# secastel/phaser

Measured on AMD Instinct MI355X. Metric: het-SNP allele calls/sec + phased variants/sec, whole-genome RNA-seq, 1→8 GPUs, higher is better.
Workload: dtype u8/int32; 1 GPU; configs[2]: whole genome (22 autosomes), one GTEx-shape RNA-seq sample, 79999998 records x 76 bp, 1499988 het SNPs, one shard per chromosome; chromosomes LPT-assigned to GPUs by record count; records=79999998, het_snps=1499988

## Files before the change

phaser_amd/csrc/phz_map.hip:

```cpp
#include "phz_internal.h"
#include "phz_lbound.h"
#include <stdlib.h>
#include <string.h>

namespace {

#ifndef PHZ_MAP_WIN
#define PHZ_MAP_WIN 512
#endif
#ifndef PHZ_CIG_X2
#define PHZ_CIG_X2 5
#endif
#ifndef PHZ_CAND_X4
#define PHZ_CAND_X4 3
#endif
constexpr int MAP_WIN = PHZ_MAP_WIN;

constexpr uint32_t OP_M = 0, OP_I = 1, OP_D = 2, OP_N = 3, OP_S = 4, OP_EQ = 7, OP_X = 8, OP_G = 9;

struct MapArgs {
    const int32_t *pos;
    const uint32_t *cigar_off, *cigar, *seq_off;
    const uint8_t *seq2, *qual;
    const uint8_t *bq;
// ... 441 lines not shown
        const int j = k * MAP_BLOCK + tid;
        const bool ok = j < nr;
        rpos_[k] = ok ? a.pos[r0 + j] : 0;
        soff_[k] = ok ? a.seq_off[r0 + j] : 0;
        coff_[k] = a.cigar_off[r0 + (ok ? j : nr)];
    }
    const uint32_t coff_end = a.cigar_off[r0 + nr];
    int v_first = 0x7fffffff;
    if (tid < vw.wlen) { const int idx = vw.w0 + tid; v_first = idx < a.nv ? a.vpos[idx] : 0x7fffffff; }
    uint32_t cg[3] = {0, 0, 0};
#pragma unroll
    for (int u = 0; u < 3; u++) { const uint32_t j = (uint32_t)tid + (uint32_t)u * MAP_BLOCK; if (j < cnt_w) cg[u] = a.cigar[cw.c_begin + j]; }
#pragma unroll
    for (int k = 0; k < RPT; k++) {
        const int j = k * MAP_BLOCK + tid;
        s_pos[j] = rpos_[k]; s_soff[j] = soff_[k]; s_coff[j] = coff_[k];
    }
    if (tid == 0) { s_coff[TILE] = coff_end; s_ncand = 0; s_ncx = 0; s_nlong = 0; s_nins = 0; }
    if (tid < TILE / 32) s_poison[tid] = 0;
    const int wdepth = window_depth(vw.wlen);
#ifdef PHZ_FILL_ALL
    const int wfill = MAP_WIN;
#else
    const int wfill = (1 << wdepth) > vw.wlen ? (1 << wdepth) : vw.wlen;
#endif
    if (tid < wfill) s_vpos[tid] = v_first;
    for (int j = tid + MAP_BLOCK; j < wfill; j += MAP_BLOCK) {
        const int idx = vw.w0 + j;
        s_vpos[j] = (j < vw.wlen && idx < a.nv) ? a.vpos[idx] : 0x7fffffff;
    }
#pragma unroll
    for (int u = 0; u < 3; u++) { const uint32_t j = (uint32_t)tid + (uint32_t)u * MAP_BLOCK; if (j < cnt_w) s_cig[j] = cg[u]; }
    for (uint32_t j = (uint32_t)tid + 3u * MAP_BLOCK; j < cnt_w; j += MAP_BLOCK) s_cig[j] = a.cigar[cw.c_begin + j];
    __syncthreads();
    PHZ_STAMP(1);
    CandBuf cb;
    cb.key = s_key; cb.var = s_var; cb.x0 = s_x0; cb.ins = s_ins; cb.n = &s_ncand; cb.nins = &s_nins; cb.cap = CAND; cb.w0 = vw.w0;
    const long long cover = (long long)s_pos[nr - 1] + MAP_COVER;

    uint32_t c0_[RPT], c1_[RPT];
    int base_[RPT], n_[RPT];
    uint32_t vmask_[RPT], codes_[RPT];
    bool fast_[RPT];
#pragma unroll
    for (int k = 0; k < RPT; k++) {
        const int j = k * MAP_BLOCK + tid;
        c0_[k] = s_coff[j]; c1_[k] = s_coff[j + 1];
        base_[k] = 0; n_[k] = 0; vmask_[k] = 0; codes_[k] = 0; fast_[k] = false;
    }
    const bool walk_on = !(a.dbg & 8);
    int len_[RPT]; bool one_[RPT];
#pragma unroll
    for (int k = 0; k < RPT; k++) {
        const int j = k * MAP_BLOCK + tid;
        one_[k] = false; len_[k] = 0;
        const uint32_t d = c0_[k] - cw.c_begin;
        if (j < nr && walk_on && complete && c1_[k] - c0_[k] == 1 && d < (uint32_t)CIG) {
            const uint32_t w = s_cig[d];
            const uint32_t op = w & 15;
            len_[k] = (int)(w >> 4);
            one_[k] = (op == OP_M || op == OP_EQ || op == OP_X) && (long long)rpos_[k] + len_[k] <= cover;
        }
    }
    constexpr int GROUP = 64 / (2 * RPT);
    int target = 0x7fffffff;
#pragma unroll
    for (int k = 0; k < RPT; k++) {
        const int e = wave_max(one_[k] ? rpos_[k] + len_[k] : (int)0x80000000);
        const int first = __builtin_amdgcn_readfirstlane(rpos_[k]);
        if ((lane / GROUP) == 2 * k) target = first;
        if ((lane / GROUP) == 2 * k + 1) target = e;
    }
    const int bound = lds_lower_bound(s_vpos, wdepth, target);
#pragma unroll
    for (int k = 0; k < RPT; k++) {
        const int j = k * MAP_BLOCK + tid;
        const int lo = __builtin_amdgcn_readlane(bound, 2 * k * GROUP), hi = __builtin_amdgcn_readlane(bound, (2 * k + 1) * GROUP);
        if (one_[k]) {
            const int pos = rpos_[k], end = pos + len_[k];
            if (hi - lo <= 24) {
                int below = 0, c = 0;
                for (int e = lo; e < hi; e++) {
                    const int vp = s_vpos[e];
                    below += vp < pos ? 1 : 0;
                    c += (vp >= pos && vp < end) ? 1 : 0;
                }
                if (c <= 8) { fast_[k] = true; base_[k] = lo + below; n_[k] = c; }
            } else {
                const int base = lds_lower_bound(s_vpos, wdepth, pos);
                int c = 0;
                while (base + c < vw.wlen && s_vpos[base + c] < end && c <= 8) c++;
                if (c <= 8) { fast_[k] = true; base_[k] = base; n_[k] = c; }
            }
        }
        if (j < nr && walk_on && !fast_[k]) {
            if (s_coff[j + 1] - s_coff[j] > 3u) s_cx[TILE - 1 - atomicAdd(&s_nlong, 1)] = (uint16_t)j;
            else s_cx[atomicAdd(&s_ncx, 1)] = (uint16_t)j;
        }
    }
    uint32_t pre_q[RPT], pre_s[RPT];
#pragma unroll
    for (int k = 0; k < RPT; k++) {
        pre_q[k] = 0; pre_s[k] = 0;
        if (fast_[k] && n_[k] > 0 && !(a.dbg & 1)) {
            const uint32_t soff = s_soff[k * MAP_BLOCK + tid];
            const int x = s_vpos[base_[k]] - rpos_[k];
            if (PHZ_ONEPLANE(a)) pre_q[k] = a.bq[(size_t)soff * 4 + x];
            else { pre_q[k] = a.qual[(size_t)soff * 4 + x]; pre_s[k] = PHZ_SEQ_BYTE(a, soff, x); }
        }
    }
    PHZ_STAMP(2);
    __syncthreads();
    PHZ_STAMP(3);
    const int nshort = walk_on ? s_ncx : 0;
    const int ncx = (walk_on && !(a.dbg & 256)) ? nshort + s_nlong : 0;
    const bool lean_on = complete && !(a.dbg & 32);
    bool redo_any = false;
    for (int t = tid; t < ncx; t += MAP_BLOCK) {
        const int ts = t < nshort ? t : TILE - 1 - (t - nshort);
        const int j = s_cx[ts];
        const bool done = lean_on && walk_lean(s_vpos, vw.wlen, wdepth, vw.w0, s_cig, cw.c_begin, (uint32_t)CIG, cb, s_poison, j, s_pos[j], s_coff[j], s_coff[j + 1], cover, a.dbg);
        if (!done) { s_cx[ts] = (uint16_t)(j | 0x8000); redo_any = true; }
    }
    const bool redo = __syncthreads_or(redo_any ? 1 : 0) != 0;
#pragma unroll
    for (int k = 0; k < RPT; k++) s_mask[k * MAP_BLOCK + tid] = 0;
    if (redo) {
        for (int t = tid; t < ncx; t += MAP_BLOCK) {
            const int jf = s_cx[t < nshort ? t : TILE - 1 - (t - nshort)];
            if (jf & 0x8000) { const int j = jf & 0x7FFF; walk_read<0>(a, vw, cw, cb, j, r0 + j, a.pos[r0 + j], s_coff[j], s_coff[j + 1], 0, 0, 0); }
        }
    }
    __syncthreads();
    PHZ_STAMP(4);
    const int ncand = s_ncand;
    const bool fb = ncand > CAND;
    uint32_t cq = 0, cs = 0; int cx_off = -1;
    if (!fb && tid < ncand && !(a.dbg & 1)) {
        const uint32_t key = s_key[tid];
        if ((key & 0xFF) == 7u) {
            const uint32_t x0 = cand_x0(cb, tid);
            cx_off = x0 != 0xFFFFFFFFu ? (int)x0 : (int)(cand_x1(cb, tid, key) >> 12);
            const uint32_t soff = s_soff[key >> 16];
            if (PHZ_ONEPLANE(a)) cq = a.bq[(size_t)soff * 4 + cx_off];
            else { cq = a.qual[(size_t)soff * 4 + cx_off]; cs = PHZ_SEQ_BYTE(a, soff, cx_off); }
        }
    }
#pragma unroll
    for (int k = 0; k < RPT; k++) {
        if (!fast_[k]) continue;
        const int j = k * MAP_BLOCK + tid;
        const uint32_t soff = s_soff[j];
        for (int o = 0; o < n_[k]; o++) {
            const int x = s_vpos[base_[k] + o] - rpos_[k];
            int sy;
            if (a.dbg & 1) sy = x & 3;
            else if (o == 0) {
                if (PHZ_ONEPLANE(a)) sy = sym_from_bq(a, soff, x, pre_q[k]);
                else {
                    const uint32_t q = pre_q[k], sb = (pre_s[k] >> (2 * (x & 3))) & 3;
                    sy = (int)(q & 0x7f) < a.baseq ? 4 : ((q & 0x80) ? (sb == 0 ? 4 : 5) : (int)sb);
                }
            } else sy = masked_base(a, soff, x);
            if (sy != 4) { vmask_[k] |= 1u << o; codes_[k] |= (uint32_t)(sy < 4 ? sy : 4) << (4 * o); }
        }
    }
    int cnt[RPT], off[RPT];
    if (!fb) {
        for (int e = tid; e < ncand; e += MAP_BLOCK) {
            uint32_t key = s_key[e];
            const int j = (int)(key >> 16);
            int code = (int)(key & 0xFF);
            if ((key & 0x8000u) && ((s_poison[j >> 5] >> (j & 31)) & 1u)) code = -1;
            else if (code == 7) {
                const uint32_t x0 = cand_x0(cb, e);
                const int x = x0 != 0xFFFFFFFFu ? (int)x0 : (int)(cand_x1(cb, e, key) >> 12);
                int sy;
                if (a.dbg & 1) sy = x & 3;
                else if (e == tid && cx_off == x) {
                    if (PHZ_ONEPLANE(a)) sy = sym_from_bq(a, s_soff[j], x, cq);
                    else {
                        const uint32_t sb = (cs >> (2 * (x & 3))) & 3;
                        sy = (int)(cq & 0x7f) < a.baseq ? 4 : ((cq & 0x80) ? (sb == 0 ? 4 : 5) : (int)sb);
                    }
                } else sy = masked_base(a, s_soff[j], x);
                code = sy < 4 ? sy : (sy == 4 ? -1 : 4);
            }
            if (code >= 0) {
                atomicOr(&s_mask[j], 1u << ((key >> 8) & 31));
                s_key[e] = (key & 0xFFFFFF00u) | (uint32_t)code;
            } else {
                s_key[e] = key | 0xFFu;
            }
        }
        __syncthreads();
#pragma unroll
        for (int k = 0; k < RPT; k++) cnt[k] = fast_[k] ? __popc(vmask_[k]) : __popc(s_mask[k * MAP_BLOCK + tid]);
    } else {
#pragma unroll
        for (int k = 0; k < RPT; k++) {
            const int j = k * MAP_BLOCK + tid;
            cnt[k] = fast_[k] ? __popc(vmask_[k])
                              : (j < nr && walk_on ? walk_read<1>(a, vw, cw, cb, j, r0 + j, rpos_[k], c0_[k], c1_[k], s_soff[j], 0, 0) : 0);
        }
    }
    PHZ_STAMP(5);
    const int T = block_scan<MAP_BLOCK, RPT>(cnt, off, s_wsum, lane, wave);
#pragma unroll
    for (int k = 0; k < RPT; k++) s_coff[k * MAP_BLOCK + tid] = (uint32_t)off[k];
    if (tid == 0) {
        a.tile_total[gtile] = T;
        uint32_t first = (uint32_t)(gtile * (int64_t)a.slot_cap);
        int room = a.slot_cap;
        if (T > a.slot_cap) {
            const OvfArea ov = *bt.ovf;
            const unsigned long long at = atomicAdd(ov.cursor, (unsigned long long)T);
            const bool fits = at + (unsigned long long)T <= (unsigned long long)ov.cap;
            if (fits) { first = (uint32_t)(ov.base + (long long)at); room = T; }
            ov.tile_first[gtile] = fits ? first : 0xFFFFFFFFu;
        }
        s_ncx = (int)first; s_nlong = room;
    }
    __syncthreads();
    PHZ_STAMP(6);
    if (a.dbg & 2) return;
    const int64_t slot0 = (int64_t)(uint32_t)s_ncx;
    const int slot_n = s_nlong;
#pragma unroll
    for (int k = 0; k < RPT; k++) {
        const int j = k * MAP_BLOCK + tid;
        if (fast_[k]) {
            int o2 = off[k];
            for (int o = 0; o < n_[k]; o++) {
                if (!((vmask_[k] >> o) & 1)) continue;
                if (o2 < slot_n) {
                    const int64_t g = slot0 + o2;
                    stage_put(a.stage, a.side, a.slots, g, (uint32_t)(vw.w0 + base_[k] + o), (uint32_t)(s_vpos[base_[k] + o] - rpos_[k]), 0u,
                              (uint32_t)j, (codes_[k] >> (4 * o)) & 15u);
                }
                o2++;
            }
        } else if (fb && cnt[k] > 0) {
            walk_read<2>(a, vw, cw, cb, j, r0 + j, rpos_[k], c0_[k], c1_[k], s_soff[j], slot0 + off[k], slot0 + slot_n);
        }
    }
    if (!fb) {
        for (int e = tid; e < ncand; e += MAP_BLOCK) {
            const uint32_t key = s_key[e];
            if ((key & 0xFF) == 0xFF) continue;
            const int j = (int)(key >> 16);
            const uint32_t ord = (key >> 8) & 31;
            const int o = (int)s_coff[j] + __popc(s_mask[j] & ((1u << ord) - 1));
            if (o < slot_n) {
                const int64_t g = slot0 + o;
                stage_put(a.stage, a.side, a.slots, g, (uint32_t)(vw.w0 + (int)s_var[e]), cand_x0(cb, e), cand_x1(cb, e, key), (uint32_t)j, key & 15u);
            }
        }
    }
    PHZ_STAMP(7);
#undef PHZ_STAMP
}

#ifndef PHZ_MAP_WAVES
#define PHZ_MAP_WAVES 8
#endif
#if PHZ_MAP_WAVES > 0
#define PHZ_MAP_OCC __attribute__((amdgpu_waves_per_eu(PHZ_MAP_WAVES, PHZ_MAP_WAVES)))
#else
#define PHZ_MAP_OCC
#endif
template <int MAP_BLOCK, int RPT, bool ABL, bool ONE = false>
__global__ __launch_bounds__(MAP_BLOCK) PHZ_MAP_OCC void k_map(MapBatch bt) {
    map_tile<MAP_BLOCK, RPT, ABL, ONE>(bt, (int64_t)blockIdx.x);
}

__global__ __launch_bounds__(1024) void k_chunk_scan(const int32_t *tile_total, int64_t ntiles, int32_t *tile_pref, int64_t *chunk_sum,
                                                     int32_t *chunk_max) {
    __shared__ int s_w[16], s_m[16];
    const int tid = threadIdx.x, lane = tid & 63, wave = tid >> 6;
    const int64_t i = (int64_t)blockIdx.x * 1024 + tid;
    const int v = i < ntiles ? tile_total[i] : 0;
    int x = v, mx = v;
#pragma unroll
    for (int d = 1; d < 64; d <<= 1) {
        int y = __shfl_up(x, d);
        if (lane >= d) x += y;
    }
#pragma unroll
    for (int d = 32; d >= 1; d >>= 1) { int y = __shfl_xor(mx, d); mx = y > mx ? y : mx; }
    if (lane == 63) s_w[wave] = x;
    if (lane == 0) s_m[wave] = mx;
    __syncthreads();
    int before = 0;
    for (int w2 = 0; w2 < wave; w2++) before += s_w[w2];
    if (i < ntiles) tile_pref[i] = before + x - v;
    if (tid == 1023) chunk_sum[blockIdx.x] = before + x;
    if (tid == 0) {
        int m = 0;
        for (int w2 = 0; w2 < 16; w2++) m = s_m[w2] > m ? s_m[w2] : m;
        chunk_max[blockIdx.x] = m;
    }
}

__global__ __launch_bounds__(1024) void k_chunk_base(const int64_t *chunk_sum, const int32_t *chunk_max, int nchunks, int64_t *chunk_base,
                                                     unsigned long long *scal ) {
    __shared__ long long s_w[16];
    __shared__ long long s_carry;
    __shared__ int s_m[16];
    const int tid = threadIdx.x, lane = tid & 63, wave = tid >> 6;
    if (tid == 0) s_carry = 0;
    int mx = 0;
    __syncthreads();
    for (int b0 = 0; b0 < nchunks; b0 += 1024) {
        const int i = b0 + tid;
        const long long v = i < nchunks ? chunk_sum[i] : 0;
        if (i < nchunks) mx = chunk_max[i] > mx ? chunk_max[i] : mx;
        long long x = v;
#pragma unroll
        for (int d = 1; d < 64; d <<= 1) {
            long long y = __shfl_up(x, d);
            if (lane >= d) x += y;
        }
        if (lane == 63) s_w[wave] = x;
        __syncthreads();
        long long before = s_carry;
        for (int w2 = 0; w2 < wave; w2++) before += s_w[w2];
        if (i < nchunks) chunk_base[i] = before + x - v;
        __syncthreads();
        if (tid == 1023) s_carry = before + x;
        __syncthreads();
    }
#pragma unroll
    for (int d = 32; d >= 1; d >>= 1) { int y = __shfl_xor(mx, d); mx = y > mx ? y : mx; }
    if (lane == 0) s_m[wave] = mx;
    __syncthreads();
    if (tid == 0) {
        int m = 0;
        for (int w2 = 0; w2 < 16; w2++) m = s_m[w2] > m ? s_m[w2] : m;
        scal[0] = (unsigned long long)s_carry;
        scal[1] = (unsigned long long)m;
    }
}

struct CompactArgs {
    const uint2 *stage; const uint32_t *side; int64_t slots;
    const ShardDev *shards; const int64_t *tile0; int n_shards;
    const int32_t *tile_total; const int32_t *tile_pref; const int64_t *chunk_base; const int64_t *shard_base;
    const int32_t *tile_w0;
    int slot_cap, tile_reads; int64_t ntiles;
    const uint32_t *tile_ovf;
};

__device__ __forceinline__ int64_t calls_before(const int64_t *chunk_base, const int32_t *tile_pref, int64_t T) {
    return chunk_base[T >> 10] + tile_pref[T];
}

__global__ void k_shard_totals(const int64_t *tile0, int n_shards, int64_t ntiles, const int32_t *tile_pref, const int64_t *chunk_base,
                               unsigned long long *scal, int64_t *shard_base) {
    const int s = blockIdx.x * blockDim.x + threadIdx.x;
    if (s >= n_shards) return;
    const int64_t a = tile0[s], b = tile0[s + 1];
    const int64_t lo = a < ntiles ? calls_before(chunk_base, tile_pref, a) : (int64_t)scal[0];
    const int64_t hi = b < ntiles ? calls_before(chunk_base, tile_pref, b) : (int64_t)scal[0];
    shard_base[s] = lo;
    scal[2 + s] = (unsigned long long)(hi - lo);
}

#ifndef PHZ_CT
#define PHZ_CT 4
#endif
constexpr int CT = PHZ_CT, CT_UNR = 4;
template <bool UNI>
__device__ __forceinline__ void compact_run(const CompactArgs &c, const int *pref, const int64_t *dstv, const int32_t *r0v, const int32_t *siv, const int64_t *slotv,
                                            int64_t T0, int M, int lane, int si0) {
    for (int e0 = lane; e0 < M; e0 += 64 * CT_UNR) {
        int k_[CT_UNR]; uint2 w_[CT_UNR]; int64_t g_[CT_UNR];
#pragma unroll
        for (int u = 0; u < CT_UNR; u++) {
            const int e = e0 + 64 * u;
            int k = 0;
#pragma unroll
            for (int st = CT / 2; st > 0; st >>= 1) k += (pref[k + st] <= e) ? st : 0;
            k_[u] = k;
            g_[u] = slotv[k] + (e - pref[k]);
            w_[u] = e < M ? c.stage[g_[u]] : make_uint2(0u, 0u);
        }
#pragma unroll
        for (int u = 0; u < CT_UNR; u++) {
            const int e = e0 + 64 * u;
            if (e >= M) break;
            const int k = k_[u];
            const uint2 w = w_[u];
            const ShardDev &sh = c.shards[UNI ? si0 : siv[k]];
            const int64_t o = dstv[k] + (e - pref[k]);
            if (o < sh.cap) {
                sh.o_read[o] = r0v[k] + (int32_t)(w.y & 0x3FFu);
                sh.o_var[o] = (int32_t)w.x;
                sh.o_code[o] = (uint8_t)((w.y >> 10) & 15u);
                if (sh.o_aux0) {
                    uint32_t a0 = w.y >> 16, a1 = 0u;
                    if (w.y & 0x8000u) a0 = c.side[g_[u]];
                    if (w.y & 0x4000u) a1 = c.side[c.slots + g_[u]];
                    sh.o_aux0[o] = a0;
                    sh.o_aux1[o] = a1;
                }
            }
        }
    }
}

__global__ __launch_bounds__(256) void k_compact(CompactArgs c) {
    __shared__ int s_pref[4][CT + 1];
    __shared__ int64_t s_dst[4][CT], s_slot[4][CT];
    __shared__ int32_t s_r0[4][CT], s_si[4][CT];
    const int w = threadIdx.x >> 6, lane = threadIdx.x & 63;
    const int64_t T0 = ((int64_t)blockIdx.x * 4 + w) * CT;
    const int64_t T = T0 + lane;
    int n = 0, si = -1;
    if (lane < CT && T < c.ntiles) {
        n = c.tile_total[T];
        int64_t first = T * (int64_t)c.slot_cap;
        if (n > c.slot_cap) {
            const uint32_t ov = c.tile_ovf[T];
            if (ov != 0xFFFFFFFFu) first = (int64_t)ov; else n = c.slot_cap;
        }
        s_slot[w][lane] = first;
        si = (c.tile_w0[4 * T + 1] >> 16) & 0x1FFF;
        s_dst[w][lane] = calls_before(c.chunk_base, c.tile_pref, T) - c.shard_base[si];
        s_r0[w][lane] = (int32_t)((T - c.tile0[si]) * c.tile_reads);
        s_si[w][lane] = si;
    }
    const int incl = wave_incl_scan(n);
    if (lane < CT) s_pref[w][lane + 1] = incl;
    if (lane == 0) s_pref[w][0] = 0;
    __syncthreads();
    const int M = __builtin_amdgcn_readlane(incl, CT - 1);
    if (M == 0) return;
    const int si0 = __builtin_amdgcn_readfirstlane(si);
    const bool uni = __ballot(si >= 0 && si != si0) == 0ull;
    if (uni) compact_run<true>(c, s_pref[w], s_dst[w], s_r0[w], s_si[w], s_slot[w], T0, M, lane, si0);
    else compact_run<false>(c, s_pref[w], s_dst[w], s_r0[w], s_si[w], s_slot[w], T0, M, lane, si0);
}

template <class T> static T *part_at(const DevBuf &b, size_t off) { return (T *)((char *)b.p + off); }

struct MapTab {
    size_t off_tile0, off_base, off_ovf;
    explicit MapTab(int m) : off_tile0((size_t)m * sizeof(ShardDev)), off_base(off_tile0 + (size_t)(m + 1) * 8), off_ovf(off_base + (size_t)m * 8) {}
    size_t table_bytes() const { return off_base; }
    size_t bytes() const { return off_ovf + 64; }
    ShardDev *shards(const DevBuf &b) const { return part_at<ShardDev>(b, 0); }
    OvfArea *ovf(const DevBuf &b) const { return part_at<OvfArea>(b, off_ovf); }
    int64_t *tile0(const DevBuf &b) const { return part_at<int64_t>(b, off_tile0); }
    int64_t *shard_base(const DevBuf &b) const { return part_at<int64_t>(b, off_base); }
};
struct MapDesc {
    size_t off_sum, off_base, off_max, bytes;
    MapDesc(int64_t ntiles, int nchunks) : off_sum(((size_t)ntiles * 4 + 15) & ~(size_t)15), off_base(off_sum + (size_t)nchunks * 8), off_max(off_base + (size_t)nchunks * 8),
                                           bytes((size_t)ntiles * 4 + (size_t)nchunks * 24 + 64) {}
    int32_t *tile_pref(const DevBuf &b) const { return part_at<int32_t>(b, 0); }
    int64_t *chunk_sum(const DevBuf &b) const { return part_at<int64_t>(b, off_sum); }
    int64_t *chunk_base(const DevBuf &b) const { return part_at<int64_t>(b, off_base); }
    int32_t *chunk_max(const DevBuf &b) const { return part_at<int32_t>(b, off_max); }
};
struct MapScalars {
    int m;
    size_t readback_bytes() const { return (size_t)8 * (m + 3); }
    size_t bytes() const { return readback_bytes() + 128; }
    unsigned long long *words(const DevBuf &b) const { return part_at<unsigned long long>(b, 0); }
    unsigned long long &shard_calls(const DevBuf &b, int k) const { return words(b)[2 + k]; }
    unsigned long long *cursor(const DevBuf &b) const { return words(b) + 2 + m; }
};

struct MapKnobs {
    int blk, rpt, dbg; unsigned dyn_lds; bool two_planes;
    static int positive(const char *name, int dflt) { const char *e = getenv(name); return e && atoi(e) > 0 ? atoi(e) : dflt; }
    MapKnobs() : blk(positive("PHZ_MAP_BLOCK", 128)), rpt(positive("PHZ_MAP_RPT", 2)), dyn_lds((unsigned)positive("PHZ_MAP_DYNLDS", 0)), two_planes(getenv("PHZ_MAP_TWO_PLANES") != nullptr) {
        const char *e = getenv("PHZ_MAP_DBG"); dbg = e ? atoi(e) : 0;
    }
};

struct MapSubmission {
    phz_ctx *ctx; hipStream_t sm; DevBuf *S;
    const int n; const phz_reads *r; const phz_variants *v; const int baseq; const phz_calls *out; int64_t *n_calls;
    const MapKnobs knobs; int tile_reads = 0;
    std::vector<int> live; std::vector<int64_t> tile0;
    int m = 0, nchunks = 0; int64_t ntiles = 0; bool one_plane = false;
    MapTab tab{0}; MapDesc desc{0, 0}; MapScalars scal{0};
    float ms_total = 0;

    MapSubmission(phz_ctx *c, int n_, const phz_reads *r_, const phz_variants *v_, int baseq_, const phz_calls *out_, int64_t *n_calls_)
        : ctx(c), sm(c->stream), S(c->scratch), n(n_), r(r_), v(v_), baseq(baseq_), out(out_), n_calls(n_calls_) {}
    template <class T> T *scr(int slot) const { return (T *)S[slot].p; }

    int live_shards_and_tiles() {
        if (!((knobs.blk == 128 || knobs.blk == 256) && knobs.rpt == 2)) return phz_fail(ctx, PHZ_E_ARG, "bad PHZ_MAP_BLOCK / PHZ_MAP_RPT");
        tile_reads = knobs.blk * knobs.rpt;
        for (int i = 0; i < n; i++) {
            if (v[i].n > 0x7fffffff) return phz_fail(ctx, PHZ_E_ARG, "too many variants in one shard");
            if (r[i].n_reads > 0 && v[i].n > 0) { live.push_back(i); tile0.push_back(ntiles); ntiles += (r[i].n_reads + tile_reads - 1) / tile_reads; }
        }
        tile0.push_back(ntiles);
        m = (int)live.size();
        if (ntiles >= (1ll << 31)) return phz_fail(ctx, PHZ_E_ARG, "too many tiles in one submission");
        if (m > 0x1FFF) return phz_fail(ctx, PHZ_E_ARG, "more than 8191 shards in one submission");
        nchunks = (int)((ntiles + 1023) / 1024);
        tab = MapTab(m); desc = MapDesc(ntiles, nchunks); scal = MapScalars{m};
        return PHZ_OK;
    }
    int shard_table() {
        auto &M = ctx->map;
        if (int s = phz_reserve_host(ctx, M.tab_host, tab.bytes())) return s;
        if (int s = phz_reserve(ctx, M.tab, tab.bytes())) return s;
        ShardDev *hs = tab.shards(M.tab_host);
        one_plane = !knobs.two_planes;
        for (int k = 0; k < m; k++) {
            const int i = live[(size_t)k];
            ShardDev &d = hs[k];
            d.pos = r[i].pos; d.cigar_off = r[i].cigar_off; d.cigar = r[i].cigar; d.seq_off = r[i].seq_off; d.seq2 = r[i].seq2; d.qual = r[i].qual; d.bq = r[i].bq;
            d.n = r[i].n_reads; d.vpos = v[i].pos; d.nv = (int)v[i].n; d.pad = 0;
            d.o_read = out[i].read_idx; d.o_var = out[i].var_idx; d.o_code = out[i].code; d.o_aux0 = out[i].aux0; d.o_aux1 = out[i].aux1;
            if (!d.o_aux0 || !d.o_aux1) { d.o_aux0 = nullptr; d.o_aux1 = nullptr; }
            d.cap = out[i].cap;
            if (!d.bq) one_plane = false;
        }
        memcpy(tab.tile0(M.tab_host), tile0.data(), (size_t)(m + 1) * 8);
        const char *img = (const char *)hs;
        if (M.tab_image.size() != tab.table_bytes() || M.tab_dev != M.tab.p || memcmp(M.tab_image.data(), img, tab.table_bytes()) != 0) {
            PHZ_HIP(ctx, hipMemcpyAsync(M.tab.p, img, tab.table_bytes(), hipMemcpyHostToDevice, sm));
            M.tab_image.assign(img, img + tab.table_bytes());
            M.tab_dev = M.tab.p;
        }
        for (hipEvent_t &e : M.ev) if (!e) PHZ_HIP(ctx, hipEventCreate(&e));
        return PHZ_OK;
    }
    int reserve() {
        auto &M = ctx->map;
        if (int s = reserve_all(ctx, {{M.tile_w0, (size_t)ntiles * 16}, {S[SC_MAP_TILE_TOTAL], (size_t)ntiles * 4}, {M.desc, desc.bytes}, {ctx->scalars, scal.bytes()}})) return s;
        if (int s = phz_reserve_host(ctx, ctx->h_scalars, scal.bytes())) return s;
        if (int s = phz_reserve(ctx, S[SC_MAP_TILE_OVF], (size_t)ntiles * 4)) return s;
        if (M.slot_cap <= 0 || M.tile_reads != tile_reads) {
            M.slot_cap = tile_reads / 2 < 64 ? 64 : tile_reads / 2; M.tile_reads = tile_reads;
            const char *e = getenv("PHZ_MAP_SLOT_CAP"); if (e && atoi(e) >= 1) M.slot_cap = atoi(e);
        }
        return PHZ_OK;
    }
    int staging_area(MapBatch &bt) {
        auto &M = ctx->map;
        const size_t base_slots = (size_t)ntiles * (size_t)M.slot_cap;
        if (M.ovf_cap < (int64_t)(base_slots / 4)) M.ovf_cap = (int64_t)(base_slots / 4);
        if (M.ovf_cap < 65536) M.ovf_cap = 65536;
        const size_t slots = base_slots + (size_t)M.ovf_cap;
        if (slots >= 0xFFFFFFF0ull) return phz_fail(ctx, PHZ_E_ARG, "K_map staging area beyond 2^32 slots: submit the shards in smaller batches");
        if (int s = phz_reserve(ctx, S[SC_MAP_STAGE], slots * 16)) return s;
        bt.stage = scr<uint2>(SC_MAP_STAGE); bt.side = (uint32_t *)(bt.stage + slots); bt.slots = (int64_t)slots;
        bt.slot_cap = M.slot_cap;
        OvfArea *h_ov = tab.ovf(M.tab_host), *d_ov = tab.ovf(M.tab);
        h_ov->tile_first = scr<uint32_t>(SC_MAP_TILE_OVF); h_ov->cursor = scal.cursor(ctx->scalars); h_ov->base = (long long)base_slots; h_ov->cap = (long long)M.ovf_cap;
        const long long img[5] = {(long long)(intptr_t)h_ov->tile_first, (long long)(intptr_t)h_ov->cursor, h_ov->base, h_ov->cap, (long long)(intptr_t)d_ov};
        if (memcmp(img, M.ovf_image, sizeof img) != 0) {
            PHZ_HIP(ctx, hipMemcpyAsync(d_ov, h_ov, sizeof(OvfArea), hipMemcpyHostToDevice, sm));
            memcpy(M.ovf_image, img, sizeof img);
        }
        bt.ovf = d_ov;
        return PHZ_OK;
    }
    template <int B, int R> void launch_k_map(const MapBatch &bt) const {
        const dim3 grid((unsigned)ntiles), block(B);
        if (bt.dbg) hipLaunchKernelGGL((k_map<B, R, true>), grid, block, knobs.dyn_lds, sm, bt);
        else if (one_plane) hipLaunchKernelGGL((k_map<B, R, false, true>), grid, block, knobs.dyn_lds, sm, bt);
        else hipLaunchKernelGGL((k_map<B, R, false>), grid, block, knobs.dyn_lds, sm, bt);
    }
    int attempt() {
        auto &M = ctx->map;
        MapBatch bt;
        bt.shards = tab.shards(M.tab); bt.tile0 = tab.tile0(M.tab); bt.n_shards = m; bt.baseq = baseq;
        bt.tile_w0 = (int32_t *)M.tile_w0.p; bt.tile_total = scr<int32_t>(SC_MAP_TILE_TOTAL); bt.ntiles = ntiles;
        if (int s = staging_area(bt)) return s;
        bt.dbg = knobs.dbg; bt.prof = nullptr;
        if (bt.dbg & 2048) { if (int s = phz_reserve(ctx, S[SC_MAP_PROFILE], (size_t)ntiles * 64)) return s; bt.prof = scr<unsigned long long>(SC_MAP_PROFILE); }
        hipLaunchKernelGGL(k_tile_window, dim3(nblk(ntiles)), dim3(256), 0, sm, bt, tile_reads);
        PHZ_HIP(ctx, hipEventRecord(M.ev[0], sm));
        if (knobs.blk == 128) launch_k_map<128, 2>(bt); else launch_k_map<256, 2>(bt);
        PHZ_HIP(ctx, hipEventRecord(M.ev[1], sm));
        int32_t *tile_pref = desc.tile_pref(M.desc); int64_t *chunk_sum = desc.chunk_sum(M.desc), *chunk_base = desc.chunk_base(M.desc); int32_t *chunk_max = desc.chunk_max(M.desc);
        unsigned long long *d_words = scal.words(ctx->scalars);
        hipLaunchKernelGGL(k_chunk_scan, dim3((unsigned)nchunks), dim3(1024), 0, sm, (const int32_t *)bt.tile_total, ntiles, tile_pref, chunk_sum, chunk_max);
        hipLaunchKernelGGL(k_chunk_base, dim3(1), dim3(1024), 0, sm, (const int64_t *)chunk_sum, (const int32_t *)chunk_max, nchunks, chunk_base, d_words);
        hipLaunchKernelGGL(k_shard_totals, dim3((unsigned)((m + 63) / 64)), dim3(64), 0, sm, bt.tile0, m, ntiles, (const int32_t *)tile_pref, (const int64_t *)chunk_base, d_words,
                           tab.shard_base(M.tab));
        CompactArgs c;
        c.stage = bt.stage; c.side = bt.side; c.slots = bt.slots;
        c.shards = bt.shards; c.tile0 = bt.tile0; c.n_shards = m;
        c.tile_total = bt.tile_total; c.tile_pref = tile_pref; c.chunk_base = chunk_base; c.shard_base = tab.shard_base(M.tab);
        c.tile_w0 = bt.tile_w0;
        c.slot_cap = bt.slot_cap; c.tile_reads = tile_reads; c.ntiles = ntiles; c.tile_ovf = scr<const uint32_t>(SC_MAP_TILE_OVF);
        hipLaunchKernelGGL(k_compact, dim3((unsigned)((ntiles + 4 * CT - 1) / (4 * CT))), dim3(256), 0, sm, c);
        PHZ_HIP(ctx, hipGetLastError());
        PHZ_HIP(ctx, hipMemcpyAsync(scal.words(ctx->h_scalars), d_words, scal.readback_bytes(), hipMemcpyDeviceToHost, sm));
        PHZ_HIP(ctx, hipStreamSynchronize(sm));
        float ms = 0;
        PHZ_HIP(ctx, hipEventElapsedTime(&ms, M.ev[0], M.ev[1]));
        if (bt.prof) if (int s = profile_report(bt.prof, ms)) return s;
        ms_total += ms;
        return PHZ_OK;
    }
    int profile_report(const unsigned long long *prof, float ms) {
        std::vector<unsigned long long> pr((size_t)ntiles * 8);
        PHZ_HIP(ctx, hipMemcpy(pr.data(), prof, pr.size() * 8, hipMemcpyDeviceToHost));
        double seg[7] = {0, 0, 0, 0, 0, 0, 0}; double life = 0;
        for (int64_t t = 0; t < ntiles; t++) { for (int k = 0; k < 7; k++) seg[k] += (double)(pr[8 * t + k + 1] - pr[8 * t + k]); life += (double)(pr[8 * t + 7] - pr[8 * t]); }
        fprintf(stderr, "[k_map profile] %lld tiles, kernel %.3f ms, tile lifetime %.2f us: stage loads -> LDS %.2f | single-run records + first gathers %.2f | barrier %.2f | "
                        "multi-op walk %.2f | candidate gathers + resolve %.2f | scan %.2f | flush %.2f us\n", (long long)ntiles, ms, life / ntiles / 100.0,
                seg[0] / ntiles / 100.0, seg[1] / ntiles / 100.0, seg[2] / ntiles / 100.0, seg[3] / ntiles / 100.0, seg[4] / ntiles / 100.0, seg[5] / ntiles / 100.0, seg[6] / ntiles / 100.0);
        return PHZ_OK;
    }
    bool overflow_area_held() const { return (int64_t)*scal.cursor(ctx->h_scalars) <= ctx->map.ovf_cap; }
    void grow_overflow_area() { const unsigned long long need = *scal.cursor(ctx->h_scalars); ctx->map.ovf_cap = (int64_t)need + (int64_t)(need / 16) + 4096; }
    int results() {
        ctx->last_ms[PHZ_T_MAP] = ms_total; ctx->total_ms[PHZ_T_MAP] += ms_total; ctx->launches[PHZ_T_MAP]++;
        int st = PHZ_OK;
        for (int k = 0; k < m; k++) {
            const int i = live[(size_t)k];
            n_calls[i] = (int64_t)scal.shard_calls(ctx->h_scalars, k);
            if (n_calls[i] > out[i].cap) st = PHZ_E_CAPACITY;
        }
        return st;
    }
};

}

static int launch_map_batch(phz_ctx *ctx, int n, const phz_reads *r, const phz_variants *v, int baseq, const phz_calls *out, int64_t *n_calls) {
    for (int i = 0; i < n; i++) n_calls[i] = 0;
    if (n <= 0) return PHZ_OK;
    MapSubmission sub(ctx, n, r, v, baseq, out, n_calls);
    if (int s = sub.live_shards_and_tiles()) return s;
    if (sub.m == 0) return PHZ_OK;
    if (int s = sub.shard_table()) return s;
    if (int s = sub.reserve()) return s;
    for (int attempt = 0; ; attempt++) {
        if (int s = sub.attempt()) return s;
        if (sub.overflow_area_held()) break;
        if (attempt == 2) return phz_fail(ctx, PHZ_E_HIP, "K_map staging overflow area did not converge");
        sub.grow_overflow_area();
    }
    return sub.results();
}

int phz_launch_map_batch(phz_ctx *ctx, int n, const phz_reads *r, const phz_variants *v, int baseq, const phz_calls *out,
                         int64_t *n_calls) {
    const int s = launch_map_batch(ctx, n, r, v, baseq, out, n_calls);
    if (s != PHZ_OK && s != PHZ_E_CAPACITY) { ctx->map.tab_image.clear(); ctx->map.tab_dev = nullptr; memset(ctx->map.ovf_image, 0, sizeof ctx->map.ovf_image); }
    return s;
}

int phz_launch_map(phz_ctx *ctx, const phz_reads &r, const phz_variants &v, int baseq, const phz_calls &out,
                   int64_t *n_calls) {
    return phz_launch_map_batch(ctx, 1, &r, &v, baseq, &out, n_calls);
}
```

Measured before the change: 15.39 billion allele calls/s.

## Merge shard totals into chunk-base kernel and write scalars directly to host

```diff
diff --git a/phaser_amd/csrc/phz_map.hip b/phaser_amd/csrc/phz_map.hip
--- a/phaser_amd/csrc/phz_map.hip
+++ b/phaser_amd/csrc/phz_map.hip
@@ -767,11 +767,35 @@
     }
 }
 
+__device__ __forceinline__ int64_t calls_before(const int64_t *chunk_base, const int32_t *tile_pref, int64_t T) {
+    return chunk_base[T >> 10] + tile_pref[T];
+}
+
+struct TotalsOut {
+    const int64_t *tile0; int n_shards; int64_t ntiles;
+    const int32_t *tile_pref;
+    int64_t *shard_base;
+    const unsigned long long *cursor;
+    unsigned long long *host;
+};
+__device__ __forceinline__ void shard_total(const TotalsOut &o, int s, const int64_t *chunk_base, int64_t total) {
+    const int64_t a = o.tile0[s], b = o.tile0[s + 1];
+    const int64_t lo = a < o.ntiles ? calls_before(chunk_base, o.tile_pref, a) : total;
+    const int64_t hi = b < o.ntiles ? calls_before(chunk_base, o.tile_pref, b) : total;
+    o.shard_base[s] = lo;
+    o.host[2 + s] = (unsigned long long)(hi - lo);
+}
+__device__ __forceinline__ void batch_words(const TotalsOut &o, unsigned long long total, unsigned long long max_tile) {
+    o.host[0] = total; o.host[1] = max_tile; o.host[2 + o.n_shards] = *o.cursor;
+}
+
+constexpr int BASE_LDS = 1024;
 __global__ __launch_bounds__(1024) void k_chunk_base(const int64_t *chunk_sum, const int32_t *chunk_max, int nchunks, int64_t *chunk_base,
-                                                     unsigned long long *scal ) {
+                                                     unsigned long long *scal, bool merged, TotalsOut o) {
     __shared__ long long s_w[16];
     __shared__ long long s_carry;
     __shared__ int s_m[16];
+    __shared__ int64_t s_base[BASE_LDS];
     const int tid = threadIdx.x, lane = tid & 63, wave = tid >> 6;
     if (tid == 0) s_carry = 0;
     int mx = 0;
@@ -790,7 +814,7 @@
         __syncthreads();
         long long before = s_carry;
         for (int w2 = 0; w2 < wave; w2++) before += s_w[w2];
-        if (i < nchunks) chunk_base[i] = before + x - v;
+        if (i < nchunks) { chunk_base[i] = before + x - v; if (merged) s_base[i] = before + x - v; }
         __syncthreads();
         if (tid == 1023) s_carry = before + x;
         __syncthreads();
@@ -799,12 +823,22 @@
     for (int d = 32; d >= 1; d >>= 1) { int y = __shfl_xor(mx, d); mx = y > mx ? y : mx; }
     if (lane == 0) s_m[wave] = mx;
     __syncthreads();
+    const long long total = s_carry;
     if (tid == 0) {
         int m = 0;
         for (int w2 = 0; w2 < 16; w2++) m = s_m[w2] > m ? s_m[w2] : m;
-        scal[0] = (unsigned long long)s_carry;
+        scal[0] = (unsigned long long)total;
         scal[1] = (unsigned long long)m;
-    }
+        if (merged) batch_words(o, (unsigned long long)total, (unsigned long long)m);
+    }
+    if (merged)
+        for (int s = tid; s < o.n_shards; s += 1024) shard_total(o, s, s_base, total);
+}
+
+__global__ void k_shard_totals(const int64_t *chunk_base, const unsigned long long *scal, TotalsOut o) {
+    const int s = blockIdx.x * blockDim.x + threadIdx.x;
+    if (s == 0) batch_words(o, scal[0], scal[1]);
+    if (s < o.n_shards) shard_total(o, s, chunk_base, (int64_t)scal[0]);
 }
 
 struct CompactArgs {
@@ -816,28 +850,16 @@
     const uint32_t *tile_ovf;
 };
 
-__device__ __forceinline__ int64_t calls_before(const int64_t *chunk_base, const int32_t *tile_pref, int64_t T) {
-    return chunk_base[T >> 10] + tile_pref[T];
-}
-
-__global__ void k_shard_totals(const int64_t *tile0, int n_shards, int64_t ntiles, const int32_t *tile_pref, const int64_t *chunk_base,
-                               unsigned long long *scal, int64_t *shard_base) {
-    const int s = blockIdx.x * blockDim.x + threadIdx.x;
-    if (s >= n_shards) return;
-    const int64_t a = tile0[s], b = tile0[s + 1];
-    const int64_t lo = a < ntiles ? calls_before(chunk_base, tile_pref, a) : (int64_t)scal[0];
-    const int64_t hi = b < ntiles ? calls_before(chunk_base, tile_pref, b) : (int64_t)scal[0];
-    shard_base[s] = lo;
-    scal[2 + s] = (unsigned long long)(hi - lo);
-}
-
 #ifndef PHZ_CT
 #define PHZ_CT 4
 #endif
 constexpr int CT = PHZ_CT, CT_UNR = 4;
-template <bool UNI>
+struct ShardOut { int32_t *o_read, *o_var; uint8_t *o_code; uint32_t *o_aux0, *o_aux1; int64_t cap; };
+__device__ __forceinline__ ShardOut shard_out(const ShardDev &sh) { return ShardOut{sh.o_read, sh.o_var, sh.o_code, sh.o_aux0, sh.o_aux1, sh.cap}; }
+
+template <bool UNI, bool AUX>
 __device__ __forceinline__ void compact_run(const CompactArgs &c, const int *pref, const int64_t *dstv, const int32_t *r0v, const int32_t *siv, const int64_t *slotv,
-                                            int64_t T0, int M, int lane, int si0) {
+                                            int M, int lane, const ShardOut &out0) {
     for (int e0 = lane; e0 < M; e0 += 64 * CT_UNR) {
         int k_[CT_UNR]; uint2 w_[CT_UNR]; int64_t g_[CT_UNR];
 #pragma unroll
@@ -856,13 +878,13 @@
             if (e >= M) break;
             const int k = k_[u];
             const uint2 w = w_[u];
-            const ShardDev &sh = c.shards[UNI ? si0 : siv[k]];
+            const ShardOut sh = UNI ? out0 : shard_out(c.shards[siv[k]]);
             const int64_t o = dstv[k] + (e - pref[k]);
             if (o < sh.cap) {
                 sh.o_read[o] = r0v[k] + (int32_t)(w.y & 0x3FFu);
                 sh.o_var[o] = (int32_t)w.x;
                 sh.o_code[o] = (uint8_t)((w.y >> 10) & 15u);
-                if (sh.o_aux0) {
+                if (AUX && sh.o_aux0) {
                     uint32_t a0 = w.y >> 16, a1 = 0u;
                     if (w.y & 0x8000u) a0 = c.side[g_[u]];
                     if (w.y & 0x4000u) a1 = c.side[c.slots + g_[u]];
@@ -874,6 +896,7 @@
     }
 }
 
+template <bool AUX>
 __global__ __launch_bounds__(256) void k_compact(CompactArgs c) {
     __shared__ int s_pref[4][CT + 1];
     __shared__ int64_t s_dst[4][CT], s_slot[4][CT];
@@ -903,8 +926,8 @@
     if (M == 0) return;
     const int si0 = __builtin_amdgcn_readfirstlane(si);
     const bool uni = __ballot(si >= 0 && si != si0) == 0ull;
-    if (uni) compact_run<true>(c, s_pref[w], s_dst[w], s_r0[w], s_si[w], s_slot[w], T0, M, lane, si0);
-    else compact_run<false>(c, s_pref[w], s_dst[w], s_r0[w], s_si[w], s_slot[w], T0, M, lane, si0);
+    if (uni) compact_run<true, AUX>(c, s_pref[w], s_dst[w], s_r0[w], s_si[w], s_slot[w], M, lane, shard_out(c.shards[si0]));
+    else compact_run<false, AUX>(c, s_pref[w], s_dst[w], s_r0[w], s_si[w], s_slot[w], M, lane, ShardOut{});
 }
 
 template <class T> static T *part_at(const DevBuf &b, size_t off) { return (T *)((char *)b.p + off); }
@@ -930,17 +953,19 @@
 };
 struct MapScalars {
     int m;
-    size_t readback_bytes() const { return (size_t)8 * (m + 3); }
-    size_t bytes() const { return readback_bytes() + 128; }
+    size_t dev_bytes() const { return (size_t)8 * 3 + 128; }
+    size_t host_bytes() const { return (size_t)8 * (m + 3) + 128; }
+    unsigned long long *dev_words(const DevBuf &b) const { return part_at<unsigned long long>(b, 0); }
+    unsigned long long *dev_cursor(const DevBuf &b) const { return dev_words(b) + 2; }
     unsigned long long *words(const DevBuf &b) const { return part_at<unsigned long long>(b, 0); }
     unsigned long long &shard_calls(const DevBuf &b, int k) const { return words(b)[2 + k]; }
     unsigned long long *cursor(const DevBuf &b) const { return words(b) + 2 + m; }
 };
 
 struct MapKnobs {
-    int blk, rpt, dbg; unsigned dyn_lds; bool two_planes;
+    int blk, rpt, dbg, merge_chunks; unsigned dyn_lds; bool two_planes;
     static int positive(const char *name, int dflt) { const char *e = getenv(name); return e && atoi(e) > 0 ? atoi(e) : dflt; }
-    MapKnobs() : blk(positive("PHZ_MAP_BLOCK", 128)), rpt(positive("PHZ_MAP_RPT", 2)), dyn_lds((unsigned)positive("PHZ_MAP_DYNLDS", 0)), two_planes(getenv("PHZ_MAP_TWO_PLANES") != nullptr) {
+    MapKnobs() : blk(positive("PHZ_MAP_BLOCK", 128)), rpt(positive("PHZ_MAP_RPT", 2)), merge_chunks(positive("PHZ_MAP_MERGE_CHUNKS", BASE_LDS)), dyn_lds((unsigned)positive("PHZ_MAP_DYNLDS", 0)), two_planes(getenv("PHZ_MAP_TWO_PLANES") != nullptr) {
         const char *e = getenv("PHZ_MAP_DBG"); dbg = e ? atoi(e) : 0;
     }
 };
@@ -950,7 +975,7 @@
     const int n; const phz_reads *r; const phz_variants *v; const int baseq; const phz_calls *out; int64_t *n_calls;
     const MapKnobs knobs; int tile_reads = 0;
     std::vector<int> live; std::vector<int64_t> tile0;
-    int m = 0, nchunks = 0; int64_t ntiles = 0; bool one_plane = false;
+    int m = 0, nchunks = 0; int64_t ntiles = 0; bool one_plane = false, text_planes = false;
     MapTab tab{0}; MapDesc desc{0, 0}; MapScalars scal{0};
     float ms_total = 0;
 
@@ -988,6 +1013,7 @@
             if (!d.o_aux0 || !d.o_aux1) { d.o_aux0 = nullptr; d.o_aux1 = nullptr; }
             d.cap = out[i].cap;
             if (!d.bq) one_plane = false;
+            if (d.o_aux0) text_planes = true;
         }
         memcpy(tab.tile0(M.tab_host), tile0.data(), (size_t)(m + 1) * 8);
         const char *img = (const char *)hs;
@@ -1001,8 +1027,8 @@
     }
     int reserve() {
         auto &M = ctx->map;
-        if (int s = reserve_all(ctx, {{M.tile_w0, (size_t)ntiles * 16}, {S[SC_MAP_TILE_TOTAL], (size_t)ntiles * 4}, {M.desc, desc.bytes}, {ctx->scalars, scal.bytes()}})) return s;
-        if (int s = phz_reserve_host(ctx, ctx->h_scalars, scal.bytes())) return s;
+        if (int s = reserve_all(ctx, {{M.tile_w0, (size_t)ntiles * 16}, {S[SC_MAP_TILE_TOTAL], (size_t)ntiles * 4}, {M.desc, desc.bytes}, {ctx->scalars, scal.dev_bytes()}})) return s;
+        if (int s = phz_reserve_host(ctx, ctx->h_scalars, scal.host_bytes())) return s;
         if (int s = phz_reserve(ctx, S[SC_MAP_TILE_OVF], (size_t)ntiles * 4)) return s;
         if (M.slot_cap <= 0 || M.tile_reads != tile_reads) {
             M.slot_cap = tile_reads / 2 < 64 ? 64 : tile_reads / 2; M.tile_reads = tile_reads;
@@ -1021,7 +1047,7 @@
         bt.stage = scr<uint2>(SC_MAP_STAGE); bt.side = (uint32_t *)(bt.stage + slots); bt.slots = (int64_t)slots;
         bt.slot_cap = M.slot_cap;
         OvfArea *h_ov = tab.ovf(M.tab_host), *d_ov = tab.ovf(M.tab);
-        h_ov->tile_first = scr<uint32_t>(SC_MAP_TILE_OVF); h_ov->cursor = scal.cursor(ctx->scalars); h_ov->base = (long long)base_slots; h_ov->cap = (long long)M.ovf_cap;
+        h_ov->tile_first = scr<uint32_t>(SC_MAP_TILE_OVF); h_ov->cursor = scal.dev_cursor(ctx->scalars); h_ov->base = (long long)base_slots; h_ov->cap = (long long)M.ovf_cap;
         const long long img[5] = {(long long)(intptr_t)h_ov->tile_first, (long long)(intptr_t)h_ov->cursor, h_ov->base, h_ov->cap, (long long)(intptr_t)d_ov};
         if (memcmp(img, M.ovf_image, sizeof img) != 0) {
             PHZ_HIP(ctx, hipMemcpyAsync(d_ov, h_ov, sizeof(OvfArea), hipMemcpyHostToDevice, sm));
@@ -1049,20 +1075,24 @@
         if (knobs.blk == 128) launch_k_map<128, 2>(bt); else launch_k_map<256, 2>(bt);
         PHZ_HIP(ctx, hipEventRecord(M.ev[1], sm));
         int32_t *tile_pref = desc.tile_pref(M.desc); int64_t *chunk_sum = desc.chunk_sum(M.desc), *chunk_base = desc.chunk_base(M.desc); int32_t *chunk_max = desc.chunk_max(M.desc);
-        unsigned long long *d_words = scal.words(ctx->scalars);
+        unsigned long long *d_words = scal.dev_words(ctx->scalars);
         hipLaunchKernelGGL(k_chunk_scan, dim3((unsigned)nchunks), dim3(1024), 0, sm, (const int32_t *)bt.tile_total, ntiles, tile_pref, chunk_sum, chunk_max);
-        hipLaunchKernelGGL(k_chunk_base, dim3(1), dim3(1024), 0, sm, (const int64_t *)chunk_sum, (const int32_t *)chunk_max, nchunks, chunk_base, d_words);
-        hipLaunchKernelGGL(k_shard_totals, dim3((unsigned)((m + 63) / 64)), dim3(64), 0, sm, bt.tile0, m, ntiles, (const int32_t *)tile_pref, (const int64_t *)chunk_base, d_words,
-                           tab.shard_base(M.tab));
+        TotalsOut to;
+        to.tile0 = bt.tile0; to.n_shards = m; to.ntiles = ntiles; to.tile_pref = tile_pref; to.shard_base = tab.shard_base(M.tab);
+        to.cursor = scal.dev_cursor(ctx->scalars); to.host = scal.words(ctx->h_scalars);
+        const bool merged = nchunks <= BASE_LDS && nchunks <= knobs.merge_chunks;
+        hipLaunchKernelGGL(k_chunk_base, dim3(1), dim3(1024), 0, sm, (const int64_t *)chunk_sum, (const int32_t *)chunk_max, nchunks, chunk_base, d_words, merged, to);
+        if (!merged) hipLaunchKernelGGL(k_shard_totals, dim3((unsigned)((m + 63) / 64)), dim3(64), 0, sm, (const int64_t *)chunk_base, (const unsigned long long *)d_words, to);
         CompactArgs c;
         c.stage = bt.stage; c.side = bt.side; c.slots = bt.slots;
         c.shards = bt.shards; c.tile0 = bt.tile0; c.n_shards = m;
         c.tile_total = bt.tile_total; c.tile_pref = tile_pref; c.chunk_base = chunk_base; c.shard_base = tab.shard_base(M.tab);
         c.tile_w0 = bt.tile_w0;
         c.slot_cap = bt.slot_cap; c.tile_reads = tile_reads; c.ntiles = ntiles; c.tile_ovf = scr<const uint32_t>(SC_MAP_TILE_OVF);
-        hipLaunchKernelGGL(k_compact, dim3((unsigned)((ntiles + 4 * CT - 1) / (4 * CT))), dim3(256), 0, sm, c);
+        const dim3 cgrid((unsigned)((ntiles + 4 * CT - 1) / (4 * CT)));
+        if (text_planes) hipLaunchKernelGGL(k_compact<true>, cgrid, dim3(256), 0, sm, c);
+        else hipLaunchKernelGGL(k_compact<false>, cgrid, dim3(256), 0, sm, c);
         PHZ_HIP(ctx, hipGetLastError());
-        PHZ_HIP(ctx, hipMemcpyAsync(scal.words(ctx->h_scalars), d_words, scal.readback_bytes(), hipMemcpyDeviceToHost, sm));
         PHZ_HIP(ctx, hipStreamSynchronize(sm));
         float ms = 0;
         PHZ_HIP(ctx, hipEventElapsedTime(&ms, M.ev[0], M.ev[1]));
```

New measurement: 16.09 billion allele calls/s (median of 6 runs). 4.6% higher.
